# yuxng/PoseCNN

Hardware: NVIDIA H100
Metric: frames/sec on 640x480 RGB, 21 classes, batch 32 (VGG16 + Hough + ROI pose head) (higher is better)
Workload: dtype bf16 operands / fp32 accumulate (conv stack, 1x1 heads), fp16 operands / fp32 accumulate (fc6-fc8), fp32 / int32 elsewhere

## Files before the change

posecnn_b200/csrc/hough_vote.cu:

```cuda
#include <float.h>
#include <stdlib.h>

#include <algorithm>

#include "common.cuh"
#include "heads_common.cuh"

namespace pcnn {
namespace hough {

constexpr int kChunk = 2048;
constexpr int kThreads = 256;
constexpr int kWarps = kThreads / 32;
constexpr int kCandCapThr = 4096;
constexpr int kMaxM = 16383;

struct __align__(16) Sample {
    int xy;
    float u, v;
    float n1;
    float k1, k2;
    int mflags;
    float d;
};
static_assert(sizeof(Sample) == 32, "sample record is two 16-byte vectors");

struct VertexSrc {
    const float* dense;
    const float* lowres;
    const float* bias;
    int h, w;
};

struct Layout {
    int nchunks, nbands, R, samp_cap, cand_cap;
    size_t chunk_hist, cls_size, cls_slot, cls_nsamp, cls_soff, slot_cls, img_count, bbox, samples, band_res, work,
        work_ctr, cand_key, cand_val, cand_n, cand_data, votes, total;
};

static int band_rows(int B, int H, int W, int C)
{
    int R = 16;
    while (R > 1 && (size_t)R * (W + 3) * 4 > 48 * 1024) R >>= 1;
    static const int forced = getenv("PCNN_HOUGH_BAND_ROWS") ? atoi(getenv("PCNN_HOUGH_BAND_ROWS")) : 0;
    if (forced >= 1 && forced <= R && (forced & (forced - 1)) == 0) return forced;
    static const int min_rows = getenv("PCNN_HOUGH_BAND_MIN") ? atoi(getenv("PCNN_HOUGH_BAND_MIN")) : 8;
    const long long want = 16LL * 4 * kNumSMs;
    while (R > min_rows && (long long)B * C * ((H + R - 1) / R) < want) R >>= 1;
    return R;
}

static Layout make_layout(int B, int H, int W, int C, int skip, bool want_votes, bool threshold_mode)
{
    Layout L;
    size_t HW = (size_t)H * W;
    L.nchunks = (int)((HW + kChunk - 1) / kChunk);
    L.R = band_rows(B, H, W, C);
    L.nbands = (H + L.R - 1) / L.R;
    L.samp_cap = (int)((HW + skip - 1) / skip) + C;
    L.cand_cap = threshold_mode ? kCandCapThr : C;
    size_t o = 0;
    auto take = [&](size_t bytes) { size_t r = o; o = align_up(o + bytes, 256); return r; };
    L.chunk_hist = take(sizeof(int) * (size_t)B * L.nchunks * C);
    L.cls_size = take(sizeof(int) * (size_t)B * C);
    L.cls_slot = take(sizeof(int) * (size_t)B * C);
    L.cls_nsamp = take(sizeof(int) * (size_t)B * C);
    L.cls_soff = take(sizeof(int) * (size_t)B * C);
    L.slot_cls = take(sizeof(int) * (size_t)B * C);
    L.img_count = take(sizeof(int) * (size_t)B);
    L.bbox = take(sizeof(int) * (size_t)B * C * 4);
    L.samples = take(sizeof(Sample) * (size_t)B * L.samp_cap);
    L.band_res = take(sizeof(int2) * (size_t)B * C * L.nbands);
    L.work = take(sizeof(int) * (size_t)B * C * L.nbands);
    L.work_ctr = take(sizeof(int) * 4);
    L.cand_key = take(sizeof(int) * (size_t)B * L.cand_cap);
    L.cand_val = take(sizeof(int) * (size_t)B * L.cand_cap);
    L.cand_n = take(sizeof(int) * (size_t)B);
    L.cand_data = take(sizeof(float4) * (size_t)B * L.cand_cap);
    L.votes = want_votes ? take(sizeof(float) * (size_t)B * C * HW) : o;
    L.total = o;
    return L;
}

__device__ __forceinline__ float project_box(int cls, const float* __restrict__ extents,
                                             const float* __restrict__ meta, float distance, float factor)
{
    float xHalf = extents[cls * 3 + 0] * 0.5f;
    float yHalf = extents[cls * 3 + 1] * 0.5f;
    float zHalf = extents[cls * 3 + 2] * 0.5f;
    float fx = meta[0], fy = meta[4], px = meta[2], py = meta[5];
    float minX = 1e8f, maxX = -1e8f, minY = 1e8f, maxY = -1e8f;
#pragma unroll
    for (int i = 0; i < 8; i++) {
        float X = (i & 1) ? -xHalf : xHalf;
        float Y = (i & 2) ? -yHalf : yHalf;
        float Z = __fadd_rn((i & 4) ? -zHalf : zHalf, distance);
        float x = __fmaf_rn(fx, __fdiv_rn(X, Z), px);
        float y = __fmaf_rn(fy, __fdiv_rn(Y, Z), py);
        minX = fminf(minX, x); minY = fminf(minY, y);
        maxX = fmaxf(maxX, x); maxY = fmaxf(maxY, y);
    }
    float width = __fadd_rn(__fsub_rn(maxX, minX), 1.f);
    float height = __fadd_rn(__fsub_rn(maxY, minY), 1.f);
    return __fmul_rn(fmaxf(width, height), factor);
}

__device__ __forceinline__ bool pred_exact(float u, float v, float n1, float dx, float dy, float inlier)
{
    float n2 = __fsqrt_rn(__fmaf_rn(dx, dx, __fmul_rn(dy, dy)));
    float dot = __fmaf_rn(u, dx, __fmul_rn(v, dy));
    float c = __fdiv_rn(dot, __fmul_rn(n1, n2));
    return c > inlier;
}

__device__ __forceinline__ bool pred_fast(float u, float v, float n1, float tn1, float dx, float dy, float vdy,
                                          float dy2, float inlier)
{
    float s2 = __fmaf_rn(dx, dx, dy2);
    float dot = __fmaf_rn(u, dx, vdy);
    float rhs = tn1 * (s2 * rsqrtf(s2));
    float g = dot - rhs;
    if (fabsf(g) > 4e-6f * rhs) return g > 0.f;
    return pred_exact(u, v, n1, dx, dy, inlier);
}

struct ZeroList {
    float* p[5];
    unsigned n[5];
};

__global__ void __launch_bounds__(kThreads)
k_hist(const int* __restrict__ label, int HW, int C, int nchunks, int* __restrict__ chunk_hist, int* __restrict__ cls_size,
       int* __restrict__ bbox, int* __restrict__ cand_n, int* __restrict__ work_ctr, ZeroList z)
{
    extern __shared__ int sh[];
    const int b = blockIdx.y, chunk = blockIdx.x, t = threadIdx.x, lane = t & 31;
    {
        unsigned gid = (blockIdx.y * gridDim.x + blockIdx.x) * kThreads + t;
        unsigned gsz = gridDim.x * gridDim.y * kThreads;
#pragma unroll
        for (int k = 0; k < 5; k++)
            for (unsigned i = gid; i < z.n[k]; i += gsz) z.p[k][i] = 0.f;
    }
    if (chunk == 0) {
        for (int c = t; c < C; c += kThreads) {
            int* bb = bbox + ((size_t)b * C + c) * 4;
            bb[0] = 0x7fffffff; bb[1] = -1; bb[2] = 0x7fffffff; bb[3] = -1;
        }
        if (t == 0) {
            cand_n[b] = 0;
            if (b == 0) { work_ctr[0] = 0; work_ctr[1] = 0; }
        }
    }
    for (int c = t; c < C; c += kThreads) sh[c] = 0;
    __syncthreads();
    const int* lab = label + (size_t)b * HW;
#pragma unroll
    for (int j = 0; j < kChunk / kThreads; j++) {
        int p = chunk * kChunk + j * kThreads + t;
        int cls = p < HW ? lab[p] : -1;
        bool valid = cls > 0 && cls < C;
        unsigned peers = __match_any_sync(0xffffffffu, valid ? cls : -1);
        if (valid && lane == __ffs(peers) - 1) atomicAdd(&sh[cls], __popc(peers));
    }
    __syncthreads();
    int* out = chunk_hist + ((size_t)b * nchunks + chunk) * C;
    for (int c = t; c < C; c += kThreads) {
        int v = sh[c];
        out[c] = v;
        if (v) atomicAdd(&cls_size[b * C + c], v);
    }
}

__global__ void __launch_bounds__(kThreads)
k_emit(const int* __restrict__ label, const VertexSrc vsrc, const float* __restrict__ extents,
       const float* __restrict__ meta_all, int H, int W, int C, int num_meta, int nchunks, int skip, int label_thr,
       float inlier, const int* __restrict__ chunk_hist, const int* __restrict__ cls_size, int* __restrict__ cls_slot,
       int* __restrict__ cls_nsamp, int* __restrict__ cls_soff, int* __restrict__ slot_cls, int* __restrict__ img_count,
       Sample* __restrict__ samples, int samp_cap, int* __restrict__ bbox)
{
    extern __shared__ int wh[];
    const int b = blockIdx.y, chunk = blockIdx.x, t = threadIdx.x, lane = t & 31, w = t >> 5;
    const int HW = H * W;
    int* sbb = wh + kWarps * C;
    int* s_slot = sbb + 4 * C;
    int* s_soff = s_slot + C;
    int* s_pref = s_soff + C;
    if (w == 0) {
        int slot_run = 0, soff_run = 0;
        for (int c0 = 0; c0 < C; c0 += 32) {
            const int c = c0 + lane;
            const int sz = c < C ? cls_size[b * C + c] : 0;
            const bool present = c > 0 && c < C && sz > label_thr;
            const int ns = present ? (sz + skip - 1) / skip : 0;
            const unsigned pm = __ballot_sync(0xffffffffu, present);
            int incl = ns;
#pragma unroll
            for (int o = 1; o < 32; o <<= 1) {
                int nb = __shfl_up_sync(0xffffffffu, incl, o);
                if (lane >= o) incl += nb;
            }
            const int slot = slot_run + __popc(pm & ((1u << lane) - 1u));
            const int soff = soff_run + incl - ns;
            if (c < C) {
                s_slot[c] = present ? slot : -1;
                s_soff[c] = soff;
                if (chunk == 0) {
                    cls_slot[b * C + c] = present ? slot : -1;
                    cls_nsamp[b * C + c] = ns;
                    cls_soff[b * C + c] = present ? soff : 0;
                    if (present) slot_cls[b * C + slot] = c;
                }
            }
            slot_run += __popc(pm);
            soff_run += __shfl_sync(0xffffffffu, incl, 31);
        }
        if (chunk == 0 && lane == 0) img_count[b] = slot_run;
    }
    for (int i = t; i < kWarps * C; i += kThreads) wh[i] = 0;
    for (int i = t; i < C; i += kThreads) { sbb[4 * i] = 0x7fffffff; sbb[4 * i + 1] = -1; sbb[4 * i + 2] = 0x7fffffff; sbb[4 * i + 3] = -1; }
    __syncthreads();
    for (int c = w; c < C; c += kWarps) {
        int sum = 0;
        if (s_slot[c] >= 0)
            for (int k = lane; k < chunk; k += 32) sum += chunk_hist[((size_t)b * nchunks + k) * C + c];
#pragma unroll
        for (int o = 16; o > 0; o >>= 1) sum += __shfl_xor_sync(0xffffffffu, sum, o);
        if (lane == 0) s_pref[c] = sum;
    }
    const int* lab = label + (size_t)b * HW;
    const int base = chunk * kChunk + w * (kChunk / kWarps);
    int labs[kChunk / kThreads];
#pragma unroll
    for (int s = 0; s < kChunk / kThreads; s++) {
        int p = base + s * 32 + lane;
        int cls = p < HW ? lab[p] : -1;
        if (!(cls > 0 && cls < C) || s_slot[cls] < 0) cls = -1;
        labs[s] = cls;
    }
#pragma unroll
    for (int s = 0; s < kChunk / kThreads; s++) {
        int cls = labs[s];
        unsigned peers = __match_any_sync(0xffffffffu, cls);
        if (cls >= 0 && lane == __ffs(peers) - 1) wh[w * C + cls] += __popc(peers);
        __syncwarp();
    }
    __syncthreads();
    for (int c = t; c < C; c += kThreads) {
        int run = s_pref[c];
#pragma unroll
        for (int ww = 0; ww < kWarps; ww++) {
            int tmp = wh[ww * C + c];
            wh[ww * C + c] = run;
            run += tmp;
        }
    }
    __syncthreads();
    const float* meta = meta_all + (size_t)b * num_meta;
    const unsigned lt = (1u << lane) - 1u;
    int2* queue = reinterpret_cast<int2*>(wh + (((kWarps + 7) * C + 1) & ~1));
    __shared__ int s_qn;
    if (t == 0) s_qn = 0;
    __syncthreads();
#pragma unroll
    for (int s = 0; s < kChunk / kThreads; s++) {
        int cls = labs[s];
        unsigned peers = __match_any_sync(0xffffffffu, cls);
        int rank = 0;
        if (cls >= 0) rank = wh[w * C + cls] + __popc(peers & lt);
        __syncwarp();
        if (cls >= 0 && lane == __ffs(peers) - 1) wh[w * C + cls] += __popc(peers);
        __syncwarp();
        if (cls >= 0 && rank % skip == 0) {
            int pos = atomicAdd(&s_qn, 1);
            queue[pos] = make_int2((w * (kChunk / kWarps) + s * 32 + lane) | (cls << 16), rank / skip);
        }
    }
    __syncthreads();
    const int qn = s_qn;
    for (int qi = t; qi < qn; qi += kThreads) {
        const int2 qe = queue[qi];
        const int cls = qe.x >> 16;
        const int p = chunk * kChunk + (qe.x & 0xffff);
        {
            int x = p % W, y = p / W;
            float u, v, z;
            if (vsrc.dense) {
                size_t off = (size_t)3 * cls + (size_t)3 * C * ((size_t)b * HW + p);
                u = vsrc.dense[off]; v = vsrc.dense[off + 1]; z = vsrc.dense[off + 2];
            } else {
                const int ch = C + 3 * cls;
                u = up8_value(vsrc.lowres, b, vsrc.h, vsrc.w, 4 * C, ch, y, x, __ldg(vsrc.bias + 3 * cls));
                v = up8_value(vsrc.lowres, b, vsrc.h, vsrc.w, 4 * C, ch + 1, y, x, __ldg(vsrc.bias + 3 * cls + 1));
                z = up8_value(vsrc.lowres, b, vsrc.h, vsrc.w, 4 * C, ch + 2, y, x, __ldg(vsrc.bias + 3 * cls + 2));
            }
            float d = expf(z);
            const float s2 = __fmaf_rn(u, u, __fmul_rn(v, v));
            float n1 = __fsqrt_rn(s2);
            float thr = project_box(cls, extents, meta, d, 0.6f);
            const bool half = n1 == 0.f && (u != 0.f || v != 0.f);
            int m = -1;
            if (thr == thr && (n1 > 0.f || half) && n1 < INFINITY) {
                float mf = fminf(fmaxf(ceilf(thr) - 1.f, -1.f), (float)kMaxM);
                m = (int)mf;
            }
            float inv = 1.f / n1, uh = u * inv, vh = v * inv;
            float ca = inlier;
            const bool sub = s2 > 0.f && s2 < FLT_MIN;
            if (sub) {
                const float us = u * 0x1p64f, vs = v * 0x1p64f, ns = sqrtf(us * us + vs * vs);
                uh = us / ns;
                vh = vs / ns;
                ca = fminf(inlier * (n1 * 0x1p64f) / ns, 1.f);
            }
            float sa = sqrtf(fmaxf(1.f - ca * ca, 0.f));
            float r1x = ca * uh - sa * vh, r1y = ca * vh + sa * uh;
            float r2x = ca * uh + sa * vh, r2y = ca * vh - sa * uh;
            float k1 = r1x / r1y, k2 = r2x / r2y;
            int flags = (r1y > 0.f ? 1 : 0) | (r1y < 0.f ? 2 : 0) | (r2y > 0.f ? 4 : 0) | (r2y < 0.f ? 8 : 0) |
                        ((r2x - r2y * k1) > 0.f ? 16 : 0) | ((r1x - r1y * k2) > 0.f ? 32 : 0) |
                        (pred_exact(u, v, n1, 1.f, 0.f, inlier) ? 64 : 0) | (pred_exact(u, v, n1, -1.f, 0.f, inlier) ? 128 : 0) |
                        (sub ? 256 : 0);
            if (half) {
                k1 = k2 = u != 0.f ? -v / u : (v > 0.f ? -INFINITY : INFINITY);
                flags = (flags & (64 | 128)) | (u != 0.f ? 1 | 2 : (v > 0.f ? 1 : 2)) | (u >= 0.f ? 16 : 0);
            }
            Sample rec;
            rec.xy = x | (y << 16);
            rec.u = u; rec.v = v; rec.n1 = n1; rec.k1 = k1; rec.k2 = k2;
            rec.mflags = (m & 0xffff) | (flags << 16);
            rec.d = d;
            Sample* dst = samples + (size_t)b * samp_cap + s_soff[cls] + qe.y;
            reinterpret_cast<float4*>(dst)[0] = reinterpret_cast<const float4*>(&rec)[0];
            reinterpret_cast<float4*>(dst)[1] = reinterpret_cast<const float4*>(&rec)[1];
            if (m >= 0) {
                atomicMin(&sbb[4 * cls + 0], max(y - m, 0));
                atomicMax(&sbb[4 * cls + 1], min(y + m, H - 1));
                atomicMin(&sbb[4 * cls + 2], max(x - m, 0));
                atomicMax(&sbb[4 * cls + 3], min(x + m, W - 1));
            }
        }
    }
    __syncthreads();
    for (int c = t; c < C; c += kThreads)
        if (sbb[4 * c + 1] >= 0) {
            int* bb = bbox + ((size_t)b * C + c) * 4;
            atomicMin(&bb[0], sbb[4 * c]);
            atomicMax(&bb[1], sbb[4 * c + 1]);
            atomicMin(&bb[2], sbb[4 * c + 2]);
            atomicMax(&bb[3], sbb[4 * c + 3]);
        }
}

__global__ void __launch_bounds__(1024)
k_worklist(int B, int C, int R, int nbands, const int* __restrict__ img_count, const int* __restrict__ slot_cls,
           const int* __restrict__ cls_nsamp, const int* __restrict__ bbox, int* __restrict__ work,
           int* __restrict__ work_ctr)
{
    __shared__ int s_cnt[64];
    __shared__ int s_base[64];
    const int n = B * C;
    if (threadIdx.x < 64) s_cnt[threadIdx.x] = 0;
    __syncthreads();
    auto bucket = [](int ns) { return 63 - min(63, ns >> 8); };
    for (int i = threadIdx.x; i < n; i += blockDim.x) {
        int b = i / C, slot = i % C;
        if (slot >= img_count[b]) continue;
        int c = slot_cls[b * C + slot];
        const int* bb = bbox + ((size_t)b * C + c) * 4;
        if (bb[1] < bb[0]) continue;
        atomicAdd(&s_cnt[bucket(cls_nsamp[b * C + c])], bb[1] / R - bb[0] / R + 1);
    }
    __syncthreads();
    if (threadIdx.x == 0) {
        int run = 0;
        for (int k = 0; k < 64; k++) { s_base[k] = run; run += s_cnt[k]; }
        work_ctr[0] = 0; work_ctr[1] = run;
    }
    __syncthreads();
    for (int i = threadIdx.x; i < n; i += blockDim.x) {
        int b = i / C, slot = i % C;
        if (slot >= img_count[b]) continue;
        int c = slot_cls[b * C + slot];
        const int* bb = bbox + ((size_t)b * C + c) * 4;
        if (bb[1] < bb[0]) continue;
        int lo = bb[0] / R, nb = bb[1] / R - lo + 1;
        int pos = atomicAdd(&s_base[bucket(cls_nsamp[b * C + c])], nb);
        for (int k = 0; k < nb; k++) work[pos + k] = (b * C + slot) * nbands + lo + k;
    }
}

__global__ void __launch_bounds__(kThreads, 4)
k_vote(int H, int W, int C, int R, int nbands, float inlier, float tau0, const int* __restrict__ slot_cls,
       const int* __restrict__ cls_nsamp, const int* __restrict__ cls_soff, const int* __restrict__ bbox,
       const Sample* __restrict__ samples, int samp_cap, const int* __restrict__ work, int* __restrict__ work_ctr,
       int2* __restrict__ band_res, float* __restrict__ votes_out)
{
    extern __shared__ int D[];
    __shared__ int s_item;
    __shared__ int s_red_val[kWarps];
    __shared__ int s_red_idx[kWarps];
    __shared__ int4 s_q[kWarps][64];
    const int t = threadIdx.x, lane = t & 31, w = t >> 5;
    const int total = work_ctr[1];
    while (true) {
        __syncthreads();
        if (t == 0) s_item = atomicAdd(&work_ctr[0], 1);
        __syncthreads();
        const int item = s_item;
        if (item >= total) break;
        const int key = work[item];
        const int band = key % nbands, bs = key / nbands, slot = bs % C, b = bs / C;
        const int c = slot_cls[b * C + slot];
        const int* bb = bbox + ((size_t)b * C + c) * 4;
        const int xlo = bb[2], xhi = bb[3];
        const int Wd = xhi - xlo + 1;
        const int stride = (Wd + 1) | 1;
        const int r0 = band * R;
        const int nrows = min(R, H - r0);
        for (int i = t; i < R * stride; i += kThreads) D[i] = 0;
        __syncthreads();

        const int ns = cls_nsamp[b * C + c];
        const Sample* S = samples + (size_t)b * samp_cap + cls_soff[b * C + c];
        int4* Q = s_q[w];
        int qn = 0;
        const unsigned lt = (1u << lane) - 1u;

        auto drain = [&](int count) {
            if (lane < count) {
                const int4 q = Q[lane];
                const Sample* rp = S + q.x;
                const float4 q0 = __ldg(reinterpret_cast<const float4*>(rp));
                const int mfl = __float_as_int(__ldg(reinterpret_cast<const float*>(rp) + 6));
                const int xy = __float_as_int(q0.x);
                const int x = xy & 0xffff, y = xy >> 16, m = (int)(short)(mfl & 0xffff);
                const int row = q.y & 0xff, mode = q.y >> 8;
                const float u = q0.y, v = q0.z, n1 = q0.w;
                const float dy = (float)(r0 + row - y);
                const int wmin = max(x - m, 0), wmax = min(x + m, W - 1);
                const float tn1 = inlier * n1, vdy = __fmul_rn(v, dy), dy2 = dy * dy;
                auto P = [&](int cx) { return pred_fast(u, v, n1, tn1, (float)(cx - x), dy, vdy, dy2, inlier); };
                int a = q.z, e = q.w;
                bool ok = true;
                if (mode & 12) {
                    ok = false;
                    if ((mode & 4) && P(a)) { e = a; ok = true; }
                    else if ((mode & 8) && P(e)) { a = e; ok = true; }
                } else {
#pragma unroll 1
                    for (int side = 0; side < 2 && ok; side++) {
                        if (!(mode & (1 << side))) continue;
                        const int o = side ? 1 : -1, lim = side ? wmax : wmin;
                        int pc = side ? e : a;
                        while (pc != lim && P(pc + o)) pc += o;
                        while ((side ? pc >= a : pc <= e) && !P(pc)) pc -= o;
                        if (side) e = pc; else a = pc;
                        ok = a <= e;
                    }
                }
                if (ok) {
                    int* Dq = D + row * stride - xlo;
                    atomicAdd(&Dq[a], 1);
                    atomicAdd(&Dq[e + 1], -1);
                }
            }
            __syncwarp();
        };

        int sidx = w * 32 + lane;
        float4 n0 = make_float4(0, 0, 0, 0), n1v = n0;
        if (sidx < ns) {
            n0 = __ldg(reinterpret_cast<const float4*>(S + sidx));
            n1v = __ldg(reinterpret_cast<const float4*>(S + sidx) + 1);
        }
        for (int sb = w * 32; sb < ns; sb += kWarps * 32) {
            const float4 q0 = n0, q1 = n1v;
            const int scur = sidx;
            sidx += kWarps * 32;
            if (sidx < ns) {
                n0 = __ldg(reinterpret_cast<const float4*>(S + sidx));
                n1v = __ldg(reinterpret_cast<const float4*>(S + sidx) + 1);
            }
            const int xy = __float_as_int(q0.x);
            const int x = xy & 0xffff, y = xy >> 16;
            const int mflags = __float_as_int(q1.z);
            const int m = (int)(short)(mflags & 0xffff);
            const int fl = mflags >> 16;
            const int row_lo = max(y - m, r0) - r0, row_hi = min(y + m, r0 + nrows - 1) - r0;
            const bool reach = scur < ns && m >= 0 && row_lo <= row_hi;
            if (!__any_sync(0xffffffffu, reach)) continue;
            const int wmin = max(x - m, 0), wmax = min(x + m, W - 1);
            const float fm2 = (fl & 256) ? 1e12f : (float)(m * m);
#pragma unroll 1
            for (int k = 0; k < R; k++) {
                const int rl = (lane + k) & (R - 1);
                const int idy = r0 + rl - y;
                int act = 0;
                int a = 0, e = 0, mode = 0;
                if (reach && rl >= row_lo && rl <= row_hi) {
                    if (idy == 0) {
                        if (fl & 64) { a = x + 1; e = wmax; act = a <= e; }
                        else if (fl & 128) { a = wmin; e = x - 1; act = a <= e; }
                    } else {
                        const bool v1 = idy > 0 ? (fl & 1) : (fl & 2);
                        const bool v2 = idy > 0 ? (fl & 4) : (fl & 8);
                        if (v1 || v2) {
                            const float dy = (float)idy;
                            const float h1 = dy * q1.x, h2 = dy * q1.y;
                            float lo, hi;
                            if (v1 && v2) { lo = fminf(h1, h2); hi = fmaxf(h1, h2); }
                            else {
                                const float hh = v1 ? h1 : h2;
                                const bool up = v1 ? (fl & 16) : (fl & 32);
                                lo = up ? hh : -1e9f;
                                hi = up ? 1e9f : hh;
                            }
                            lo = fminf(fmaxf(lo, -40000.f), 40000.f);
                            hi = fminf(fmaxf(hi, -40000.f), 40000.f);
                            a = x + (int)ceilf(lo);
                            e = x + (int)floorf(hi);
                            const float tau = tau0 + 2e-6f * __fdividef(dy * dy + fm2, fabsf(dy));
                            if (a > e) {
                                const bool ca = (float)(a - x) - hi < tau && a >= wmin && a <= wmax;
                                const bool ce = lo - (float)(e - x) < tau && e >= wmin && e <= wmax;
                                if (ca || ce) { act = 2; mode = (ca ? 4 : 0) | (ce ? 8 : 0); }
                            } else {
                                const float ma = (float)(a - x) - lo, me = hi - (float)(e - x);
                                const bool va = a >= wmin && (ma < tau || ma > 1.f - tau);
                                const bool ve = e <= wmax && (me < tau || me > 1.f - tau);
                                const int chk = (va || ve) ? 1 : 0;
                                a = max(a, wmin);
                                e = min(e, wmax);
                                if (a <= e + chk) { act = 1 + chk; mode = (va ? 1 : 0) | (ve ? 2 : 0); }
                            }
                        }
                    }
                }
                if (act == 1) {
                    int* Drow = D + rl * stride - xlo;
                    atomicAdd(&Drow[a], 1);
                    atomicAdd(&Drow[e + 1], -1);
                }
                const unsigned need = __ballot_sync(0xffffffffu, act == 2);
                if (need) {
                    if (act == 2) Q[qn + __popc(need & lt)] = make_int4(scur, rl | (mode << 8), a, e);
                    qn += __popc(need);
                    __syncwarp();
                    if (qn >= 32) {
                        drain(32);
                        if (lane < qn - 32) Q[lane] = Q[32 + lane];
                        qn -= 32;
                        __syncwarp();
                    }
                }
            }
        }
        if (qn > 0) drain(qn);
        __syncthreads();

        int best_val = -1, best_idx = 0x7fffffff;
        for (int row = w; row < nrows; row += kWarps) {
            int carry = 0;
            int* Dr = D + row * stride;
            for (int x0 = 0; x0 < Wd; x0 += 32) {
                int xi = x0 + lane;
                int val = xi < Wd ? Dr[xi] : 0;
#pragma unroll
                for (int o = 1; o < 32; o <<= 1) {
                    int nb = __shfl_up_sync(0xffffffffu, val, o);
                    if (lane >= o) val += nb;
                }
                val += carry;
                carry = __shfl_sync(0xffffffffu, val, 31);
                if (xi < Wd) {
                    if (votes_out) Dr[xi] = val;
                    int idx = (r0 + row) * W + xlo + xi;
                    if (val > best_val) { best_val = val; best_idx = idx; }
                }
            }
        }
#pragma unroll
        for (int o = 16; o > 0; o >>= 1) {
            int ov = __shfl_xor_sync(0xffffffffu, best_val, o);
            int oi = __shfl_xor_sync(0xffffffffu, best_idx, o);
            if (ov > best_val || (ov == best_val && oi < best_idx)) { best_val = ov; best_idx = oi; }
        }
        if (lane == 0) { s_red_val[w] = best_val; s_red_idx[w] = best_idx; }
        __syncthreads();
        if (t == 0) {
            int bv = s_red_val[0], bi = s_red_idx[0];
            for (int k = 1; k < kWarps; k++)
                if (s_red_val[k] > bv || (s_red_val[k] == bv && s_red_idx[k] < bi)) { bv = s_red_val[k]; bi = s_red_idx[k]; }
            band_res[(size_t)(b * C + slot) * nbands + band] = make_int2(bv, bi);
        }
        if (votes_out) {
            float* plane = votes_out + ((size_t)b * C + c) * H * W;
            for (int i = t; i < nrows * W; i += kThreads) {
                int row = i / W, x = i % W;
                float val = (x >= xlo && x <= xhi) ? (float)D[row * stride + x - xlo] : 0.f;
                plane[(size_t)(r0 + row) * W + x] = val;
            }
        }
    }
}

__global__ void k_select(int C, int HW, int R, int nbands, int cap, int cand_cap, const int* __restrict__ img_count,
                         const int* __restrict__ slot_cls, const int* __restrict__ bbox,
                         const int2* __restrict__ band_res, int* __restrict__ cand_key, int* __restrict__ cand_val,
                         int* __restrict__ cand_n)
{
    const int b = blockIdx.x;
    const int count = img_count[b];
    const int n = min(min(count, cap), cand_cap);
    for (int slot = threadIdx.x; slot < n; slot += blockDim.x) {
        int c = slot_cls[b * C + slot];
        const int* bb = bbox + ((size_t)b * C + c) * 4;
        int bv = 0, bi = 0;
        if (bb[1] >= bb[0]) {
            int lo = bb[0] / R, hi = bb[1] / R;
            bv = -1; bi = 0x7fffffff;
            for (int k = lo; k <= hi; k++) {
                int2 r = band_res[(size_t)(b * C + slot) * nbands + k];
                if (r.x > bv || (r.x == bv && r.y < bi)) { bv = r.x; bi = r.y; }
            }
            if (bv <= 0) { bv = 0; bi = 0; }
        }
        cand_key[(size_t)b * cand_cap + slot] = slot * HW + bi;
        cand_val[(size_t)b * cand_cap + slot] = bv;
    }
    if (threadIdx.x == 0) cand_n[b] = n;
}

__global__ void __launch_bounds__(kThreads)
k_localmax(int H, int W, int C, int R, float vote_thr, int cand_cap, const int* __restrict__ img_count,
           const int* __restrict__ slot_cls, const int* __restrict__ bbox, const float* __restrict__ votes,
           int* __restrict__ cand_key, int* __restrict__ cand_val, int* __restrict__ cand_n, int* __restrict__ status)
{
    const int b = blockIdx.z, slot = blockIdx.y;
    if (slot >= img_count[b]) return;
    const int c = slot_cls[b * C + slot];
    const int* bb = bbox + ((size_t)b * C + c) * 4;
    if (bb[1] < bb[0]) return;
    const int ylo = (bb[0] / R) * R, yhi = min(H - 1, (bb[1] / R) * R + R - 1);
    const int p = blockIdx.x * kThreads + threadIdx.x;
    if (p >= H * W) return;
    const int cx = p % W, cy = p / W;
    if (cy < ylo || cy > yhi) return;
    const float* plane = votes + ((size_t)b * C + c) * H * W;
    const float val = plane[p];
    if (!(val > vote_thr)) return;
    for (int x = cx - 3; x <= cx + 3; x++)
        for (int y = cy - 3; y <= cy + 3; y++)
            if (x >= 0 && x < W && y >= ylo && y <= yhi && plane[y * W + x] > val) return;
    int pos = atomicAdd(&cand_n[b], 1);
    if (pos < cand_cap) {
        cand_key[(size_t)b * cand_cap + pos] = slot * (H * W) + p;
        cand_val[(size_t)b * cand_cap + pos] = (int)val;
    } else if (status) {
        atomicOr(&status[0], 1);
    }
}

__global__ void __launch_bounds__(kThreads)
k_celldata(int B, int H, int W, int C, int num_meta, float inlier, int cand_cap, const float* __restrict__ extents,
           const float* __restrict__ meta_all, const int* __restrict__ slot_cls, const int* __restrict__ cls_nsamp,
           const int* __restrict__ cls_soff, const Sample* __restrict__ samples, int samp_cap,
           const int* __restrict__ cand_key, const int* __restrict__ cand_n, float4* __restrict__ cand_data)
{
    __shared__ float s_sum[kThreads];
    __shared__ int s_cnt[kThreads];
    __shared__ float s_thr2;
    const int t = threadIdx.x;
    const int HW = H * W;
    {
        const int b = blockIdx.y;
        const int n = min(cand_n[b], cand_cap);
        for (int i = blockIdx.x; i < n; i += gridDim.x) {
            const int key = cand_key[(size_t)b * cand_cap + i];
            const int slot = key / HW, p = key % HW;
            const int c = slot_cls[b * C + slot];
            const int cx = p % W, cy = p / W;
            const int ns = cls_nsamp[b * C + c];
            const Sample* S = samples + (size_t)b * samp_cap + cls_soff[b * C + c];
            float sum = 0.f;
            int cnt = 0;
            for (int s = t; s < ns; s += kThreads) {
                const Sample q = S[s];
                const int x = q.xy & 0xffff, y = q.xy >> 16;
                const int m = (int)(short)(q.mflags & 0xffff);
                if (m < 0 || abs(x - cx) > m || abs(y - cy) > m) continue;
                if (pred_exact(q.u, q.v, q.n1, (float)(cx - x), (float)(cy - y), inlier)) { cnt++; sum += q.d; }
            }
            s_sum[t] = sum; s_cnt[t] = cnt;
            __syncthreads();
            for (int o = kThreads / 2; o > 0; o >>= 1) {
                if (t < o) { s_sum[t] += s_sum[t + o]; s_cnt[t] += s_cnt[t + o]; }
                __syncthreads();
            }
            const int votes = s_cnt[0];
            float dist = 0.f;
            if (votes > 0) dist = __fdiv_rn(s_sum[0], (float)votes);
            if (t == 0) s_thr2 = votes > 0 ? project_box(c, extents, meta_all + (size_t)b * num_meta, dist, 0.6f) : 0.f;
            __syncthreads();
            const float thr2 = s_thr2;
            float bbw = -1.f, bbh = -1.f;
// ... 133 lines not shown
        const float scale = 0.05f;
        const int nrow = is_train ? 9 : 1;
        const int roi = r * nrow;
        float* b0 = top_box + (size_t)roi * 7;
        const double f = 0.5 + (double)scale;
        b0[0] = (float)(b + batch_offset);
        b0[1] = (float)cls;
        b0[2] = (float)((double)x - (double)bb_width * f);
        b0[3] = (float)((double)y - (double)bb_height * f);
        b0[4] = (float)((double)x + (double)bb_width * f);
        b0[5] = (float)((double)y + (double)bb_height * f);
        b0[6] = votes;
        for (int k = 0; k < nrow; k++) {
            float* q = top_pose + (size_t)(roi + k) * 7;
            q[0] = 1.f; q[1] = 0.f; q[2] = 0.f; q[3] = 0.f;
            q[4] = __fmul_rn(rx, bb_distance); q[5] = __fmul_rn(ry, bb_distance); q[6] = bb_distance;
            if (is_train) top_domain[roi + k] = num_gt == 0 ? 1 : 0;
        }
        if (!is_train) continue;
        for (int g = 0; g < num_gt; g++) {
            const float* gp = gt + (size_t)g * 13;
            if (cls == (int)gp[1] && b + batch_offset == (int)gp[0]) {
                if (box_overlap(cls, extents, meta, gp, b0 + 2) > 0.2f) {
                    for (int j = 0; j < 9; j++)
                        for (int k = 0; k < 4; k++) {
                            top_target[(size_t)(roi + j) * 4 * C + 4 * cls + k] = gp[6 + k];
                            top_weight[(size_t)(roi + j) * 4 * C + 4 * cls + k] = 1.f;
                        }
                    break;
                }
            }
        }
        const float x1 = b0[2], y1 = b0[3], x2 = b0[4], y2 = b0[5];
        const float ww = x2 - x1, hh = y2 - y1;
        const int jx[8] = {-1, 1, -1, 1, 0, -1, 0, 1};
        const int jy[8] = {-1, -1, 1, 1, -1, 0, 1, 0};
#pragma unroll
        for (int j = 0; j < 8; j++) {
            float* q = top_box + (size_t)(roi + 1 + j) * 7;
            q[0] = (float)(b + batch_offset);
            q[1] = (float)cls;
            q[2] = jx[j] == 0 ? x1 : (float)((double)x1 + jx[j] * (0.05 * (double)ww));
            q[3] = jy[j] == 0 ? y1 : (float)((double)y1 + jy[j] * (0.05 * (double)hh));
            q[4] = q[2] + ww;
            q[5] = q[3] + hh;
            q[6] = votes;
        }
    }
}

__global__ void k_zero2(float* a, size_t na, float* b, size_t nb)
{
    size_t i = (size_t)blockIdx.x * blockDim.x + threadIdx.x, g = (size_t)gridDim.x * blockDim.x;
    for (size_t k = i; k < na / 4; k += g) reinterpret_cast<float4*>(a)[k] = make_float4(0, 0, 0, 0);
    for (size_t k = na / 4 * 4 + i; k < na; k += g) a[k] = 0.f;
    for (size_t k = i; k < nb / 4; k += g) reinterpret_cast<float4*>(b)[k] = make_float4(0, 0, 0, 0);
    for (size_t k = nb / 4 * 4 + i; k < nb; k += g) b[k] = 0.f;
}

static int run_front(const Layout& L, char* ws, const int32_t* label, const VertexSrc vertex, const float* extents,
                     const float* meta, int B, int H, int W, int C, int num_meta, float inlier, int label_thr, int skip,
                     ZeroList z, float* votes_out, cudaStream_t st)
{
    int* chunk_hist = (int*)(ws + L.chunk_hist);
    int* cls_size = (int*)(ws + L.cls_size);
    int* cls_slot = (int*)(ws + L.cls_slot);
    int* cls_nsamp = (int*)(ws + L.cls_nsamp);
    int* cls_soff = (int*)(ws + L.cls_soff);
    int* slot_cls = (int*)(ws + L.slot_cls);
    int* img_count = (int*)(ws + L.img_count);
    int* bbox = (int*)(ws + L.bbox);
    Sample* samples = (Sample*)(ws + L.samples);
    int2* band_res = (int2*)(ws + L.band_res);
    int* work = (int*)(ws + L.work);
    int* work_ctr = (int*)(ws + L.work_ctr);
    int* cand_n = (int*)(ws + L.cand_n);
    const int HW = H * W;
    dim3 grid(L.nchunks, B);
    cudaMemsetAsync(cls_size, 0, sizeof(int) * (size_t)B * C, st);
    k_hist<<<grid, kThreads, sizeof(int) * C, st>>>(label, HW, C, L.nchunks, chunk_hist, cls_size, bbox, cand_n, work_ctr, z);
    const size_t emit_smem = sizeof(int) * ((((kWarps + 7) * C + 1) & ~1) + 2 * kChunk);
    k_emit<<<grid, kThreads, emit_smem, st>>>(label, vertex, extents, meta, H, W, C, num_meta, L.nchunks, skip, label_thr,
                                              inlier, chunk_hist, cls_size, cls_slot, cls_nsamp, cls_soff, slot_cls,
                                              img_count, samples, L.samp_cap, bbox);
    k_worklist<<<1, 1024, 0, st>>>(B, C, L.R, L.nbands, img_count, slot_cls, cls_nsamp, bbox, work, work_ctr);
    size_t smem = sizeof(int) * (size_t)L.R * (W + 3);
    PCNN_SMEM_OPTIN(k_vote, 110 * 1024, "hough k_vote");
    static const float tau0 = getenv("PCNN_HOUGH_TAU0") ? (float)atof(getenv("PCNN_HOUGH_TAU0")) : 0.004f;
    k_vote<<<4 * kNumSMs, kThreads, smem, st>>>(H, W, C, L.R, L.nbands, inlier, tau0, slot_cls, cls_nsamp, cls_soff, bbox,
                                                samples, L.samp_cap, work, work_ctr, band_res, votes_out);
    return check_launch("hough front kernels");
}

static int validate(int B, int H, int W, int C, int skip)
{
    PCNN_REQUIRE(B >= 1 && H >= 1 && W >= 1 && C >= 2, "hough: need B,H,W >= 1 and C >= 2 (got %d,%d,%d,%d)", B, H, W, C);
    PCNN_REQUIRE(H <= 16383 && W <= 16383, "hough: image larger than 16383 x 16383 unsupported (got %d x %d)", W, H);
    PCNN_REQUIRE((long long)C * H * W < 0x7fffffffLL, "hough: C*H*W must fit int32 (reference flat index, .cu.cc:260)");
    PCNN_REQUIRE(skip >= 1, "hough: skip_pixels must be >= 1 (got %d)", skip);
    PCNN_REQUIRE(C <= 512, "hough: at most 512 classes supported (got %d)", C);
    return PCNN_OK;
}

}
}

using namespace pcnn;
using namespace pcnn::hough;

extern "C" int pcnn_hough_vote_workspace_bytes(int B, int H, int W, int C, int skip_pixels, float threshold_vote,
                                               size_t* bytes)
{
    int rc = validate(B, H, W, C, skip_pixels);
    if (rc) return rc;
    PCNN_REQUIRE(bytes != nullptr, "hough: bytes is NULL");
    const bool thr_mode = threshold_vote > 0;
    Layout L = make_layout(B, H, W, C, skip_pixels, thr_mode, thr_mode);
    *bytes = L.total + align_up(sizeof(int) * ((size_t)B * PCNN_MAX_ROI + B + 1), 256);
    return PCNN_OK;
}

static int hough_fwd_impl(const int32_t* label, const VertexSrc vsrc, const float* extents, const float* meta,
                          const float* gt, int B, int batch_global, int batch_offset, int H, int W, int C, int num_gt,
                          int num_meta, int is_train, float inlier_threshold, int label_threshold, float threshold_vote,
                          float threshold_percentage, int skip_pixels, float* top_box, float* top_pose,
                          float* top_target, float* top_weight, int32_t* top_domain, int32_t* num_rois,
                          int32_t* status, void* workspace, size_t workspace_bytes, void* stream)
{
    int rc = validate(B, H, W, C, skip_pixels);
    if (rc) return rc;
    PCNN_REQUIRE(is_train >= 0, "Need is_train >= 0, got %d", is_train);
    PCNN_REQUIRE(num_meta >= 6, "hough: meta_data needs the intrinsics (num_meta >= 6, got %d)", num_meta);
    PCNN_REQUIRE(num_gt == 0 || gt != nullptr, "hough: gt is NULL but num_gt = %d", num_gt);
    PCNN_REQUIRE(label && (vsrc.dense || (vsrc.lowres && vsrc.bias)) && extents && meta && top_box && top_pose &&
                     top_target && top_weight && top_domain && num_rois && workspace, "hough: NULL tensor pointer");
    PCNN_REQUIRE(batch_global >= B && batch_offset >= 0 && batch_offset + B <= batch_global,
                 "hough: shard [%d, %d) does not lie inside the global batch of %d images", batch_offset, batch_offset + B,
                 batch_global);
    const bool thr_mode = threshold_vote > 0;
    size_t need = 0;
    pcnn_hough_vote_workspace_bytes(B, H, W, C, skip_pixels, threshold_vote, &need);
    if (workspace_bytes < need) {
        set_error("hough: workspace too small (%zu < %zu)", workspace_bytes, need);
        return PCNN_E_WORKSPACE;
    }
    cudaStream_t st = (cudaStream_t)stream;
    Layout L = make_layout(B, H, W, C, skip_pixels, thr_mode, thr_mode);
    char* ws = (char*)workspace;
    int* sel = (int*)(ws + L.total);
    int* sel_n = sel + (size_t)B * PCNN_MAX_ROI;
    ZeroList z;
    const unsigned rows = PCNN_HOUGH_MAX_ROWS;
    z.p[0] = top_box; z.n[0] = rows * 7;
    z.p[1] = top_pose; z.n[1] = rows * 7;
    z.p[2] = top_target; z.n[2] = rows * 4 * C;
    z.p[3] = top_weight; z.n[3] = rows * 4 * C;
    z.p[4] = reinterpret_cast<float*>(top_domain); z.n[4] = rows;
    if (status) cudaMemsetAsync(status, 0, 4 * sizeof(int), st);
    float* votes = thr_mode ? (float*)(ws + L.votes) : nullptr;
    rc = run_front(L, ws, label, vsrc, extents, meta, B, H, W, C, num_meta, inlier_threshold, label_threshold,
                   skip_pixels, z, votes, st);
    if (rc) return rc;
    int* img_count = (int*)(ws + L.img_count);
    int* slot_cls = (int*)(ws + L.slot_cls);
    int* bbox = (int*)(ws + L.bbox);
    int* cand_key = (int*)(ws + L.cand_key);
    int* cand_val = (int*)(ws + L.cand_val);
    int* cand_n = (int*)(ws + L.cand_n);
    float4* cand_data = (float4*)(ws + L.cand_data);
    const int cap = PCNN_MAX_ROI / batch_global;
    if (!thr_mode) {
        k_select<<<B, 32, 0, st>>>(C, H * W, L.R, L.nbands, cap, L.cand_cap, img_count, slot_cls, bbox,
                                   (const int2*)(ws + L.band_res), cand_key, cand_val, cand_n);
    } else {
        dim3 g((H * W + kThreads - 1) / kThreads, C - 1, B);
        k_localmax<<<g, kThreads, 0, st>>>(H, W, C, L.R, threshold_vote, L.cand_cap, img_count, slot_cls, bbox, votes,
                                           cand_key, cand_val, cand_n, status);
    }
    dim3 gcell(thr_mode ? 64 : (unsigned)std::max(1, std::min(std::min(cap, C), L.cand_cap)), B);
    k_celldata<<<gcell, kThreads, 0, st>>>(B, H, W, C, num_meta, inlier_threshold, L.cand_cap, extents, meta, slot_cls,
                                             (const int*)(ws + L.cls_nsamp), (const int*)(ws + L.cls_soff),
                                             (const Sample*)(ws + L.samples), L.samp_cap, cand_key, cand_n, cand_data);
    k_finalize<<<1, kThreads, 0, st>>>(B, batch_offset, H, W, C, num_meta, num_gt, is_train, cap, L.cand_cap,
                                       thr_mode ? 1 : 0, threshold_percentage, extents, meta, gt, slot_cls, cand_key, cand_val,
                                       cand_n, cand_data, sel, sel_n, top_box, top_pose, top_target, top_weight, top_domain,
                                       num_rois, status);
    return check_launch("hough back kernels");
}

extern "C" int pcnn_hough_vote_fwd(const int32_t* label, const float* vertex, const float* extents, const float* meta,
                                   const float* gt, int B, int H, int W, int C, int num_gt, int num_meta, int is_train,
                                   float inlier_threshold, int label_threshold, float threshold_vote,
                                   float threshold_percentage, int skip_pixels, float* top_box, float* top_pose,
                                   float* top_target, float* top_weight, int32_t* top_domain, int32_t* num_rois,
                                   int32_t* status, void* workspace, size_t workspace_bytes, void* stream)
{
    VertexSrc vs = {vertex, nullptr, nullptr, 0, 0};
    return hough_fwd_impl(label, vs, extents, meta, gt, B, B, 0, H, W, C, num_gt, num_meta, is_train, inlier_threshold,
                          label_threshold, threshold_vote, threshold_percentage, skip_pixels, top_box, top_pose, top_target,
                          top_weight, top_domain, num_rois, status, workspace, workspace_bytes, stream);
}

extern "C" int pcnn_hough_vote_fwd_ex(const int32_t* label, const float* vertex, const float* lowres,
                                      const float* bias_vertex, const float* extents, const float* meta, const float* gt,
                                      int B, int batch_global, int batch_offset, int H, int W, int C, int num_gt,
                                      int num_meta, int is_train, float inlier_threshold, int label_threshold,
                                      float threshold_vote, float threshold_percentage, int skip_pixels, float* top_box,
                                      float* top_pose, float* top_target, float* top_weight, int32_t* top_domain,
                                      int32_t* num_rois, int32_t* status, void* workspace, size_t workspace_bytes,
                                      void* stream)
{
    PCNN_REQUIRE(vertex || (H % 8 == 0 && W % 8 == 0), "hough: the lowres vertex source needs H, W multiples of 8 (got %d x %d)", H, W);
    VertexSrc vs = {vertex, vertex ? nullptr : lowres, vertex ? nullptr : bias_vertex, H / 8, W / 8};
    return hough_fwd_impl(label, vs, extents, meta, gt, B, batch_global, batch_offset, H, W, C, num_gt, num_meta, is_train,
                          inlier_threshold, label_threshold, threshold_vote, threshold_percentage, skip_pixels, top_box,
                          top_pose, top_target, top_weight, top_domain, num_rois, status, workspace, workspace_bytes, stream);
}

extern "C" int pcnn_hough_vote_planes(const int32_t* label, const float* vertex, const float* extents, const float* meta,
                                      int B, int H, int W, int C, int num_meta, float inlier_threshold,
                                      int label_threshold, int skip_pixels, float* votes, void* workspace,
                                      size_t workspace_bytes, void* stream)
{
    int rc = validate(B, H, W, C, skip_pixels);
    if (rc) return rc;
    PCNN_REQUIRE(label && vertex && extents && meta && votes && workspace, "hough planes: NULL tensor pointer");
    Layout L = make_layout(B, H, W, C, skip_pixels, false, false);
    if (workspace_bytes < L.total) {
        set_error("hough planes: workspace too small (%zu < %zu)", workspace_bytes, L.total);
        return PCNN_E_WORKSPACE;
    }
    cudaStream_t st = (cudaStream_t)stream;
    cudaMemsetAsync(votes, 0, sizeof(float) * (size_t)B * C * H * W, st);
    ZeroList z;
    for (int k = 0; k < 5; k++) { z.p[k] = nullptr; z.n[k] = 0; }
    VertexSrc vs = {vertex, nullptr, nullptr, 0, 0};
    return run_front(L, (char*)workspace, label, vs, extents, meta, B, H, W, C, num_meta, inlier_threshold,
                     label_threshold, skip_pixels, z, votes, st);
}

extern "C" int pcnn_hough_vote_bwd(float* grad_label, float* grad_vertex, int B, int H, int W, int C, void* stream)
{
    PCNN_REQUIRE(grad_label && grad_vertex, "hough bwd: NULL pointer");
    size_t na = (size_t)B * H * W, nb = na * 3 * C;
    k_zero2<<<4 * kNumSMs, 256, 0, (cudaStream_t)stream>>>(grad_label, na, grad_vertex, nb);
    return check_launch("hough bwd");
}
```

Before: 2919.

## Cap Hough voting to ROI-limited classes and compact reaching samples per warp

Only the first cap = PCNN_MAX_ROI/batch_global present classes per image take part in voting. Samples, worklist items and band results are emitted and indexed only for those slots, and the band height is recomputed for the smaller class count. Inside k_vote, each warp now compacts the samples whose vertical span reaches the current band into a shared queue and processes them in full 32-lane batches, which reduces idle lanes. The cost is extra shared memory, ballot and queue bookkeeping, and dependence on the cap matching how many classes the selection step would have kept.

```diff
diff --git a/posecnn_b200/csrc/hough_vote.cu b/posecnn_b200/csrc/hough_vote.cu
--- a/posecnn_b200/csrc/hough_vote.cu
+++ b/posecnn_b200/csrc/hough_vote.cu
@@ -34,6 +34,7 @@
 
 struct Layout {
     int nchunks, nbands, R, samp_cap, cand_cap;
+    int nvote;
     size_t chunk_hist, cls_size, cls_slot, cls_nsamp, cls_soff, slot_cls, img_count, bbox, samples, band_res, work,
         work_ctr, cand_key, cand_val, cand_n, cand_data, votes, total;
 };
@@ -50,12 +51,16 @@
     return R;
 }
 
-static Layout make_layout(int B, int H, int W, int C, int skip, bool want_votes, bool threshold_mode)
+static Layout make_layout(int B, int H, int W, int C, int skip, bool want_votes, bool threshold_mode, int vote_cap)
 {
     Layout L;
     size_t HW = (size_t)H * W;
     L.nchunks = (int)((HW + kChunk - 1) / kChunk);
-    L.R = band_rows(B, H, W, C);
+    const int R_all = band_rows(B, H, W, C);
+    const int nbands_all = (H + R_all - 1) / R_all;
+    L.nvote = std::min(C, vote_cap);
+    L.R = band_rows(B, H, W, L.nvote);
+    if ((long long)L.nvote * ((H + L.R - 1) / L.R) > (long long)C * nbands_all) L.R = R_all;
     L.nbands = (H + L.R - 1) / L.R;
     L.samp_cap = (int)((HW + skip - 1) / skip) + C;
     L.cand_cap = threshold_mode ? kCandCapThr : C;
@@ -70,8 +75,8 @@
     L.img_count = take(sizeof(int) * (size_t)B);
     L.bbox = take(sizeof(int) * (size_t)B * C * 4);
     L.samples = take(sizeof(Sample) * (size_t)B * L.samp_cap);
-    L.band_res = take(sizeof(int2) * (size_t)B * C * L.nbands);
-    L.work = take(sizeof(int) * (size_t)B * C * L.nbands);
+    L.band_res = take(sizeof(int2) * (size_t)B * C * nbands_all);
+    L.work = take(sizeof(int) * (size_t)B * C * nbands_all);
     L.work_ctr = take(sizeof(int) * 4);
     L.cand_key = take(sizeof(int) * (size_t)B * L.cand_cap);
     L.cand_val = take(sizeof(int) * (size_t)B * L.cand_cap);
@@ -177,7 +182,7 @@
        const float* __restrict__ meta_all, int H, int W, int C, int num_meta, int nchunks, int skip, int label_thr,
        float inlier, const int* __restrict__ chunk_hist, const int* __restrict__ cls_size, int* __restrict__ cls_slot,
        int* __restrict__ cls_nsamp, int* __restrict__ cls_soff, int* __restrict__ slot_cls, int* __restrict__ img_count,
-       Sample* __restrict__ samples, int samp_cap, int* __restrict__ bbox)
+       Sample* __restrict__ samples, int samp_cap, int* __restrict__ bbox, int nvote)
 {
     extern __shared__ int wh[];
     const int b = blockIdx.y, chunk = blockIdx.x, t = threadIdx.x, lane = t & 31, w = t >> 5;
@@ -192,18 +197,19 @@
             const int c = c0 + lane;
             const int sz = c < C ? cls_size[b * C + c] : 0;
             const bool present = c > 0 && c < C && sz > label_thr;
-            const int ns = present ? (sz + skip - 1) / skip : 0;
             const unsigned pm = __ballot_sync(0xffffffffu, present);
+            const int slot = slot_run + __popc(pm & ((1u << lane) - 1u));
+            const bool voted = present && slot < nvote;
+            const int ns = voted ? (sz + skip - 1) / skip : 0;
             int incl = ns;
 #pragma unroll
             for (int o = 1; o < 32; o <<= 1) {
                 int nb = __shfl_up_sync(0xffffffffu, incl, o);
                 if (lane >= o) incl += nb;
             }
-            const int slot = slot_run + __popc(pm & ((1u << lane) - 1u));
             const int soff = soff_run + incl - ns;
             if (c < C) {
-                s_slot[c] = present ? slot : -1;
+                s_slot[c] = voted ? slot : -1;
                 s_soff[c] = soff;
                 if (chunk == 0) {
                     cls_slot[b * C + c] = present ? slot : -1;
@@ -353,18 +359,18 @@
 }
 
 __global__ void __launch_bounds__(1024)
-k_worklist(int B, int C, int R, int nbands, const int* __restrict__ img_count, const int* __restrict__ slot_cls,
+k_worklist(int B, int C, int nvote, int R, int nbands, const int* __restrict__ img_count, const int* __restrict__ slot_cls,
            const int* __restrict__ cls_nsamp, const int* __restrict__ bbox, int* __restrict__ work,
            int* __restrict__ work_ctr)
 {
     __shared__ int s_cnt[64];
     __shared__ int s_base[64];
-    const int n = B * C;
+    const int n = B * nvote;
     if (threadIdx.x < 64) s_cnt[threadIdx.x] = 0;
     __syncthreads();
     auto bucket = [](int ns) { return 63 - min(63, ns >> 8); };
     for (int i = threadIdx.x; i < n; i += blockDim.x) {
-        int b = i / C, slot = i % C;
+        int b = i / nvote, slot = i % nvote;
         if (slot >= img_count[b]) continue;
         int c = slot_cls[b * C + slot];
         const int* bb = bbox + ((size_t)b * C + c) * 4;
@@ -379,19 +385,19 @@
     }
     __syncthreads();
     for (int i = threadIdx.x; i < n; i += blockDim.x) {
-        int b = i / C, slot = i % C;
+        int b = i / nvote, slot = i % nvote;
         if (slot >= img_count[b]) continue;
         int c = slot_cls[b * C + slot];
         const int* bb = bbox + ((size_t)b * C + c) * 4;
         if (bb[1] < bb[0]) continue;
         int lo = bb[0] / R, nb = bb[1] / R - lo + 1;
         int pos = atomicAdd(&s_base[bucket(cls_nsamp[b * C + c])], nb);
-        for (int k = 0; k < nb; k++) work[pos + k] = (b * C + slot) * nbands + lo + k;
+        for (int k = 0; k < nb; k++) work[pos + k] = (b * nvote + slot) * nbands + lo + k;
     }
 }
 
 __global__ void __launch_bounds__(kThreads, 4)
-k_vote(int H, int W, int C, int R, int nbands, float inlier, float tau0, const int* __restrict__ slot_cls,
+k_vote(int H, int W, int C, int nvote, int R, int nbands, float inlier, float tau0, const int* __restrict__ slot_cls,
        const int* __restrict__ cls_nsamp, const int* __restrict__ cls_soff, const int* __restrict__ bbox,
        const Sample* __restrict__ samples, int samp_cap, const int* __restrict__ work, int* __restrict__ work_ctr,
        int2* __restrict__ band_res, float* __restrict__ votes_out)
@@ -401,6 +407,7 @@
     __shared__ int s_red_val[kWarps];
     __shared__ int s_red_idx[kWarps];
     __shared__ int4 s_q[kWarps][64];
+    __shared__ int s_sq[kWarps][64];
     const int t = threadIdx.x, lane = t & 31, w = t >> 5;
     const int total = work_ctr[1];
     while (true) {
@@ -410,7 +417,7 @@
         const int item = s_item;
         if (item >= total) break;
         const int key = work[item];
-        const int band = key % nbands, bs = key / nbands, slot = bs % C, b = bs / C;
+        const int band = key % nbands, bs = key / nbands, slot = bs % nvote, b = bs / nvote;
         const int c = slot_cls[b * C + slot];
         const int* bb = bbox + ((size_t)b * C + c) * 4;
         const int xlo = bb[2], xhi = bb[3];
@@ -468,28 +475,21 @@
             __syncwarp();
         };
 
-        int sidx = w * 32 + lane;
-        float4 n0 = make_float4(0, 0, 0, 0), n1v = n0;
-        if (sidx < ns) {
-            n0 = __ldg(reinterpret_cast<const float4*>(S + sidx));
-            n1v = __ldg(reinterpret_cast<const float4*>(S + sidx) + 1);
-        }
-        for (int sb = w * 32; sb < ns; sb += kWarps * 32) {
-            const float4 q0 = n0, q1 = n1v;
-            const int scur = sidx;
-            sidx += kWarps * 32;
-            if (sidx < ns) {
-                n0 = __ldg(reinterpret_cast<const float4*>(S + sidx));
-                n1v = __ldg(reinterpret_cast<const float4*>(S + sidx) + 1);
-            }
+        auto span = [&](int y, int m, int fl, int& lo, int& hi) {
+            const int top = (fl & (2 | 8)) ? y - m : ((fl & (64 | 128)) ? y : y + 1);
+            const int bot = (fl & (1 | 4)) ? y + m : ((fl & (64 | 128)) ? y : y - 1);
+            lo = max(top, r0) - r0;
+            hi = min(bot, r0 + nrows - 1) - r0;
+            return m >= 0 && lo <= hi;
+        };
+        auto walk = [&](bool has, int scur, const float4 q0, const float4 q1) {
             const int xy = __float_as_int(q0.x);
             const int x = xy & 0xffff, y = xy >> 16;
             const int mflags = __float_as_int(q1.z);
             const int m = (int)(short)(mflags & 0xffff);
             const int fl = mflags >> 16;
-            const int row_lo = max(y - m, r0) - r0, row_hi = min(y + m, r0 + nrows - 1) - r0;
-            const bool reach = scur < ns && m >= 0 && row_lo <= row_hi;
-            if (!__any_sync(0xffffffffu, reach)) continue;
+            int row_lo, row_hi;
+            const bool reach = has && span(y, m, fl, row_lo, row_hi);
             const int wmin = max(x - m, 0), wmax = min(x + m, W - 1);
             const float fm2 = (fl & 256) ? 1e12f : (float)(m * m);
 #pragma unroll 1
@@ -555,6 +555,48 @@
                     }
                 }
             }
+        };
+
+        int* SQ = s_sq[w];
+        int sqn = 0;
+        int sidx = w * 32 + lane;
+        float4 n0 = make_float4(0, 0, 0, 0), n1v = n0;
+        if (sidx < ns) {
+            n0 = __ldg(reinterpret_cast<const float4*>(S + sidx));
+            n1v = __ldg(reinterpret_cast<const float4*>(S + sidx) + 1);
+        }
+        for (int sb = w * 32; sb < ns || sqn > 0; sb += kWarps * 32) {
+            if (sb < ns) {
+                const float4 q0 = n0, q1 = n1v;
+                const int scur = sidx;
+                sidx += kWarps * 32;
+                if (sidx < ns) {
+                    n0 = __ldg(reinterpret_cast<const float4*>(S + sidx));
+                    n1v = __ldg(reinterpret_cast<const float4*>(S + sidx) + 1);
+                }
+                const int mflags = __float_as_int(q1.z);
+                int lo, hi;
+                const bool reach =
+                    scur < ns && span(__float_as_int(q0.x) >> 16, (int)(short)(mflags & 0xffff), mflags >> 16, lo, hi);
+                const unsigned rm = __ballot_sync(0xffffffffu, reach);
+                if (reach) SQ[sqn + __popc(rm & lt)] = scur;
+                sqn += __popc(rm);
+                __syncwarp();
+            }
+            if (sqn >= 32 || (sqn > 0 && sb + kWarps * 32 >= ns)) {
+                const bool has = lane < sqn;
+                const int s = has ? SQ[lane] : 0;
+                __syncwarp();
+                if (lane < sqn - 32) SQ[lane] = SQ[32 + lane];
+                sqn = max(sqn - 32, 0);
+                __syncwarp();
+                float4 q0 = make_float4(0, 0, 0, 0), q1 = q0;
+                if (has) {
+                    q0 = __ldg(reinterpret_cast<const float4*>(S + s));
+                    q1 = __ldg(reinterpret_cast<const float4*>(S + s) + 1);
+                }
+                walk(has, s, q0, q1);
+            }
         }
         if (qn > 0) drain(qn);
         __syncthreads();
@@ -592,7 +634,7 @@
             int bv = s_red_val[0], bi = s_red_idx[0];
             for (int k = 1; k < kWarps; k++)
                 if (s_red_val[k] > bv || (s_red_val[k] == bv && s_red_idx[k] < bi)) { bv = s_red_val[k]; bi = s_red_idx[k]; }
-            band_res[(size_t)(b * C + slot) * nbands + band] = make_int2(bv, bi);
+            band_res[(size_t)(b * nvote + slot) * nbands + band] = make_int2(bv, bi);
         }
         if (votes_out) {
             float* plane = votes_out + ((size_t)b * C + c) * H * W;
@@ -605,7 +647,7 @@
     }
 }
 
-__global__ void k_select(int C, int HW, int R, int nbands, int cap, int cand_cap, const int* __restrict__ img_count,
+__global__ void k_select(int C, int nvote, int HW, int R, int nbands, int cap, int cand_cap, const int* __restrict__ img_count,
                          const int* __restrict__ slot_cls, const int* __restrict__ bbox,
                          const int2* __restrict__ band_res, int* __restrict__ cand_key, int* __restrict__ cand_val,
                          int* __restrict__ cand_n)
@@ -621,7 +663,7 @@
             int lo = bb[0] / R, hi = bb[1] / R;
             bv = -1; bi = 0x7fffffff;
             for (int k = lo; k <= hi; k++) {
-                int2 r = band_res[(size_t)(b * C + slot) * nbands + k];
+                int2 r = band_res[(size_t)(b * nvote + slot) * nbands + k];
                 if (r.x > bv || (r.x == bv && r.y < bi)) { bv = r.x; bi = r.y; }
             }
             if (bv <= 0) { bv = 0; bi = 0; }
@@ -921,12 +963,12 @@
     const size_t emit_smem = sizeof(int) * ((((kWarps + 7) * C + 1) & ~1) + 2 * kChunk);
     k_emit<<<grid, kThreads, emit_smem, st>>>(label, vertex, extents, meta, H, W, C, num_meta, L.nchunks, skip, label_thr,
                                               inlier, chunk_hist, cls_size, cls_slot, cls_nsamp, cls_soff, slot_cls,
-                                              img_count, samples, L.samp_cap, bbox);
-    k_worklist<<<1, 1024, 0, st>>>(B, C, L.R, L.nbands, img_count, slot_cls, cls_nsamp, bbox, work, work_ctr);
+                                              img_count, samples, L.samp_cap, bbox, L.nvote);
+    k_worklist<<<1, 1024, 0, st>>>(B, C, L.nvote, L.R, L.nbands, img_count, slot_cls, cls_nsamp, bbox, work, work_ctr);
     size_t smem = sizeof(int) * (size_t)L.R * (W + 3);
     PCNN_SMEM_OPTIN(k_vote, 110 * 1024, "hough k_vote");
     static const float tau0 = getenv("PCNN_HOUGH_TAU0") ? (float)atof(getenv("PCNN_HOUGH_TAU0")) : 0.004f;
-    k_vote<<<4 * kNumSMs, kThreads, smem, st>>>(H, W, C, L.R, L.nbands, inlier, tau0, slot_cls, cls_nsamp, cls_soff, bbox,
+    k_vote<<<4 * kNumSMs, kThreads, smem, st>>>(H, W, C, L.nvote, L.R, L.nbands, inlier, tau0, slot_cls, cls_nsamp, cls_soff, bbox,
                                                 samples, L.samp_cap, work, work_ctr, band_res, votes_out);
     return check_launch("hough front kernels");
 }
@@ -954,7 +996,7 @@
     if (rc) return rc;
     PCNN_REQUIRE(bytes != nullptr, "hough: bytes is NULL");
     const bool thr_mode = threshold_vote > 0;
-    Layout L = make_layout(B, H, W, C, skip_pixels, thr_mode, thr_mode);
+    Layout L = make_layout(B, H, W, C, skip_pixels, thr_mode, thr_mode, C);
     *bytes = L.total + align_up(sizeof(int) * ((size_t)B * PCNN_MAX_ROI + B + 1), 256);
     return PCNN_OK;
 }
@@ -984,7 +1026,8 @@
         return PCNN_E_WORKSPACE;
     }
     cudaStream_t st = (cudaStream_t)stream;
-    Layout L = make_layout(B, H, W, C, skip_pixels, thr_mode, thr_mode);
+    const int cap = PCNN_MAX_ROI / batch_global;
+    Layout L = make_layout(B, H, W, C, skip_pixels, thr_mode, thr_mode, thr_mode ? C : cap);
     char* ws = (char*)workspace;
     int* sel = (int*)(ws + L.total);
     int* sel_n = sel + (size_t)B * PCNN_MAX_ROI;
@@ -1007,9 +1050,8 @@
     int* cand_val = (int*)(ws + L.cand_val);
     int* cand_n = (int*)(ws + L.cand_n);
     float4* cand_data = (float4*)(ws + L.cand_data);
-    const int cap = PCNN_MAX_ROI / batch_global;
     if (!thr_mode) {
-        k_select<<<B, 32, 0, st>>>(C, H * W, L.R, L.nbands, cap, L.cand_cap, img_count, slot_cls, bbox,
+        k_select<<<B, 32, 0, st>>>(C, L.nvote, H * W, L.R, L.nbands, cap, L.cand_cap, img_count, slot_cls, bbox,
                                    (const int2*)(ws + L.band_res), cand_key, cand_val, cand_n);
     } else {
         dim3 g((H * W + kThreads - 1) / kThreads, C - 1, B);
@@ -1064,7 +1106,7 @@
     int rc = validate(B, H, W, C, skip_pixels);
     if (rc) return rc;
     PCNN_REQUIRE(label && vertex && extents && meta && votes && workspace, "hough planes: NULL tensor pointer");
-    Layout L = make_layout(B, H, W, C, skip_pixels, false, false);
+    Layout L = make_layout(B, H, W, C, skip_pixels, false, false, C);
     if (workspace_bytes < L.total) {
         set_error("hough planes: workspace too small (%zu < %zu)", workspace_bytes, L.total);
         return PCNN_E_WORKSPACE;
```

Measured after the change: 2922 (median of 6 runs). Within noise of the previous version (+0.1%).
